# hyperpape/needle

Hardware: AMD Instinct MI355X
Metric: GB/s haystack scanned (10M x 256-char batch, DFA table walk) (higher is better)
Workload: dtype u8; 1 GPU; c2: '[0-9]+' containedIn() over 10000000 x 256 ASCII rows; rows_total=10000000, rows_per_gpu=10000000, row_chars=256, char_bytes=1, parallelism=row-shard x1, launch=eager

## Files before the change

### needle_amd/csrc/needle_device.h

```cpp
#pragma once
#include <stdint.h>

namespace needle {

enum Op : int { OP_MATCHES = 0, OP_CONTAINED_IN = 1, OP_FIND = 2 };

enum Mode : int {
    MODE_PACK = 0,
    MODE_TABLE8 = 1,
    MODE_TABLE16 = 2,
    MODE_GLOBAL = 3,
    MODE_HYBRID = 5,
    MODE_SPARSE = 6,
    MODE_PAIR = 4,
};

struct ProgHeader {
    uint32_t mode;
    uint32_t n_states;
    uint32_t n_cols;
    uint32_t start;
    uint32_t accept_lo;
    uint32_t root_accepting;
    uint32_t lds_bytes;
    uint32_t off_f;
    uint32_t pad_f;
    uint32_t pre_f;
    uint32_t off_cmap;
    uint32_t off_ptab;
    uint32_t off_pages;
    uint32_t off_table;
    uint32_t n_pages;
    uint32_t pad_col;
    uint32_t off_bcmap, off_bptab, off_bpages;
    uint32_t off_btable;
    uint8_t pack_off[8];
    uint32_t start_off, accept_off, ident_fn;
    uint32_t bpack_start_off, bpack_accept_off;
    uint32_t hot_bytes;
    uint32_t off_gtable;
    uint32_t off_bsp_bm;
    uint32_t off_bsp_base, off_bsp_edges;
    uint32_t sp_rec_base, sp_accept_rec, sp_rows_base;
    uint32_t sp_chains;
    uint32_t sp_pad_ident;
    uint32_t sp_dense, sp_records;
    uint32_t win_on, win_lo_e, win_hi_e;
    uint32_t fa_len_off, fa_dead_lo, fa_dead_n;
    uint32_t fa_dead_hi, sp_end_col4, sp_dead_row0, sp_len_cols;
    uint32_t fa_skip_lo;
    uint32_t flat_pages;
    uint32_t ft_on, ft_codes_off, ft_odd, ft_direct;
    uint32_t off_bpack;
};

struct ScanArgs {
    const uint8_t *rows;
    uint64_t n_rows;
    uint64_t stride_bytes;
    uint64_t total_bytes;
    uint32_t row_len;
    const uint32_t *lengths;
    const int32_t *from;
    const uint8_t *prog;
    ProgHeader hdr;
    const uint8_t *bprog;
    ProgHeader bhdr;
    int32_t fixed_len;
    uint32_t tiles_in_f_rows;
    uint64_t *bitmap;
    int32_t *start;
    int32_t *end;
    uint32_t *packed;
    uint32_t packed8;
    uint32_t *end_state;
    uint32_t short_window;
    uint32_t defer_max_live;
};

struct PackedArgs {
    ScanArgs s;
    const uint64_t *offsets;
    int32_t *overflow;
};

struct SpecArgs {
    const uint8_t *rows;
    uint64_t n_rows;
    uint64_t stride_bytes;
    uint32_t stripe_bytes;
    uint32_t spr;
    uint32_t char_width;
    uint32_t op;
    uint32_t row_len;
    const uint32_t *lengths;
    const uint8_t *gprog;
    ProgHeader hdr;
    uint32_t *slen;
    const uint32_t *spec_end_state;
    const int32_t *spec_last;
    const uint64_t *spec_bitmap;
    uint32_t *entry;
    uint32_t *entry_done;
    uint32_t *true_end_state;
    int32_t *true_last;
    int32_t *changed;
    uint64_t *bitmap;
    int32_t *end;
};

constexpr uint32_t kStripeBytes = 4096;
struct StripeArgs {
    const uint8_t *rows;
    uint64_t n_rows;
    uint64_t stride_bytes;
    uint32_t row_len;
    const uint32_t *lengths;
    const uint8_t *prog;
    ProgHeader hdr;
    uint32_t spr;
    uint32_t *fn;
    uint64_t *bitmap;
    uint32_t *cand;
    int32_t *cand_stripe;
    int32_t *end;
    int32_t *start;
    const uint8_t *bprog;
    ProgHeader bhdr;
    int32_t fixed_len;
    uint32_t op;
};

__host__ __device__ inline uint16_t pack8(int32_t s, int32_t e) {
    if (e < 0) return 0xFFFFu;
    const uint32_t len = (uint32_t)(e - s);
    return len > 255u ? (uint16_t)0xFFFEu : (uint16_t)(((uint32_t)s & 0xFFu) | len << 8);
}
constexpr uint32_t kPack16Over = 0xFFFEFFFFu;
constexpr uint16_t kPack8Over = 0xFFFDu;
__host__ __device__ inline uint32_t pack16_or_over(int32_t s, int32_t e) {
    if (e < 0) return 0xFFFFFFFFu;
    return e <= 65534 ? (((uint32_t)s & 0xFFFFu) | (uint32_t)e << 16) : kPack16Over;
}
__host__ __device__ inline uint16_t pack8_or_over(int32_t s, int32_t e) {
    if (e < 0) return 0xFFFFu;
    return e <= 256 ? pack8(s, e) : kPack8Over;
}
constexpr uint32_t kLdsF1 = 0, kLdsCmap1 = 0, kLdsTable1 = 512;
constexpr uint32_t kLdsCmapB1 = 512, kLdsPairTable1 = 1024;
constexpr uint32_t kLdsPtab2 = 0;
constexpr uint32_t kLdsPagesF2 = 2048, kLdsPages2Table = 512;
constexpr uint32_t kMaxPackPagesBytes = 96u * 1024u;

constexpr int kWavesPerBlock = 16;
constexpr uint32_t kMaxProgLdsBytes = 160u * 1024u - 4u * 64u * 64u;

}
```

### needle_amd/csrc/needle_kernels.hip

```cpp
#include "needle_walk.h"

namespace needle {

struct LaunchShape {
    int grid, waves, chb;
    size_t lds;
};
hipError_t launch_scan_matches(const ScanArgs &a, int cw, bool guard, LaunchShape sh, hipStream_t s);
hipError_t launch_scan_contained_in(const ScanArgs &a, int cw, bool guard, LaunchShape sh, hipStream_t s);
hipError_t launch_scan_find(const ScanArgs &a, int cw, bool guard, LaunchShape sh, hipStream_t s);

bool shape_for_program(const ProgHeader &h, int char_width, int *waves, int *chb, int *tiles_in_f_rows) {
    const size_t p = (h.lds_bytes + 15u) & ~15u;
    const size_t cap = 160u * 1024u;
    *tiles_in_f_rows = 0;
    static const char *force = getenv("NEEDLE_SHAPE");
    if (force) {
        int w = 0, c = 0;
        if (sscanf(force, "%dx%d", &w, &c) == 2 && (c == 64 || c == 128) && w >= 1 && w <= 16 && p + (size_t)w * 64 * c <= cap) {
            *waves = w;
            *chb = c;
            return true;
        }
    }
    if (h.mode == MODE_PACK && char_width == 1) {
        static const int min_waves = getenv("NEEDLE_PACK_WAVES") ? atoi(getenv("NEEDLE_PACK_WAVES")) : 14;
        for (int w = 16; w >= min_waves && w >= 5; --w)
            if (p + (size_t)(w - 4) * 8192u <= cap) {
                *waves = w;
                *chb = 128;
                *tiles_in_f_rows = 1;
                return true;
            }
    }
    static const int cand[8][2] = {{16, 128}, {12, 128}, {16, 64}, {14, 64}, {12, 64}, {10, 64}, {8, 64}, {4, 64}};
    for (const auto &c : cand) {
        if (p + (size_t)c[0] * 64 * c[1] <= cap) {
            *waves = c[0];
            *chb = c[1];
            return true;
        }
    }
    return false;
}

hipError_t launch_short_rows(int op, int char_width, const ScanArgs &a, int n_cus, hipStream_t stream);

hipError_t launch_scan(int op, int char_width, const ScanArgs &a_in, int n_cus, hipStream_t stream) {
    if (a_in.n_rows == 0) return hipSuccess;
    {
        static const int short_rows = getenv("NEEDLE_SHORT_ROWS") ? atoi(getenv("NEEDLE_SHORT_ROWS")) : 1;
        if (short_rows && a_in.stride_bytes <= 64 && a_in.hdr.mode != MODE_HYBRID && a_in.hdr.mode != MODE_SPARSE)
            return launch_short_rows(op, char_width, a_in, n_cus, stream);
    }
    ScanArgs a = a_in;
    LaunchShape sh;
    int in_f = 0;
    if (!shape_for_program(a.hdr, char_width, &sh.waves, &sh.chb, &in_f)) return hipErrorInvalidValue;
    a.tiles_in_f_rows = (uint32_t)in_f;
    const uint64_t n_groups = (a.n_rows + 63) >> 6;
    uint64_t blocks = (n_groups + sh.waves - 1) / sh.waves;
    static const int reserve = getenv("NEEDLE_RESERVE_CUS") ? atoi(getenv("NEEDLE_RESERVE_CUS")) : 0;
    if (reserve > 0 && n_cus > reserve + 8) n_cus -= reserve;
    if (blocks > (uint64_t)n_cus) blocks = (uint64_t)n_cus;
    sh.grid = (int)blocks;
    sh.lds = ((a.hdr.lds_bytes + 15u) & ~15u) + (size_t)(sh.waves - (in_f ? 4 : 0)) * 64 * sh.chb;
    static const int defer_env = getenv("NEEDLE_DEFER") ? atoi(getenv("NEEDLE_DEFER")) : 16;
    a.defer_max_live = 0;
    if (defer_env > 0 && defer_env <= 32 && !a.from && !a.end_state && a.n_rows < (1ull << 32)) a.defer_max_live = (uint32_t)defer_env;
    const bool guard = a.lengths != nullptr || a.from != nullptr || a.row_len == 0 ||
                       ((uint64_t)a.row_len * char_width) % sh.chb != 0;
    switch (op) {
    case OP_MATCHES: return launch_scan_matches(a, char_width, guard, sh, stream);
    case OP_CONTAINED_IN: return launch_scan_contained_in(a, char_width, guard, sh, stream);
    default: return launch_scan_find(a, char_width, guard, sh, stream);
    }
}

}
```

### needle_amd/csrc/needle_scan.h

```cpp
#pragma once
#include "needle_walk.h"

namespace needle {

template <int OP, int CW, int MODE, bool GUARD, int CHB, bool LEN = false>
__global__ __launch_bounds__(kWavesPerBlock * 64) void scan_kernel(const ScanArgs a) {
    using G = Geom<CHB>;
    constexpr bool POOL = MODE != MODE_PACK && CHB == 64;
    const int tid = threadIdx.x;
    const int lane = tid & 63;
    const int wave = __builtin_amdgcn_readfirstlane(tid >> 6);
    const int n_waves = blockDim.x >> 6;

    if ((uint32_t)(uintptr_t)(__attribute__((address_space(3))) unsigned char *)smem != 0u) __builtin_trap();
    for (uint32_t i = tid * 16u; i < a.hdr.lds_bytes; i += blockDim.x * 16u)
        *(u32x4 *)(smem + i) = *(const u32x4 *)(a.prog + i);
    __syncthreads();

    Walk wk;
    constexpr uint32_t ELEM = (MODE == MODE_TABLE16 || MODE == MODE_HYBRID) ? 2u : 1u;
    wk.ncols_e = a.hdr.n_cols * ELEM;
    wk.pad_e = (MODE == MODE_PACK) ? a.hdr.pad_f : a.hdr.pad_col * ELEM;
    wk.pre_e = (MODE == MODE_PACK) ? a.hdr.pre_f : (a.hdr.pad_col + 1u) * ELEM;
    wk.pad_b = wk.pre_b = 0;
    if (MODE == MODE_PAIR) {
        wk.ncols_e = a.hdr.n_cols * a.hdr.n_cols * 2u;
        wk.pad_e = a.hdr.pad_col * a.hdr.n_cols * 2u;
        wk.pre_e = (a.hdr.pad_col + 1u) * a.hdr.n_cols * 2u;
        wk.pad_b = a.hdr.pad_col * 2u;
        wk.pre_b = (a.hdr.pad_col + 1u) * 2u;
    }
    if (MODE == MODE_SPARSE) wk.pad_e = wk.pre_e = a.hdr.win_lo_e;
    wk.win_on = a.hdr.win_on;
    wk.win_lo = a.hdr.win_lo_e;
    wk.win_hi = a.hdr.win_hi_e;
    wk.dead_hi = OP == OP_FIND ? a.hdr.fa_dead_hi : 0u;
    wk.sp_chains = a.hdr.sp_chains;
    wk.sp_pad_ident = a.hdr.sp_pad_ident;
    wk.flat = (CW == 2 && (MODE == MODE_TABLE8 || MODE == MODE_TABLE16)) ? a.hdr.flat_pages : 0u;
    wk.table_off = a.hdr.off_table - (MODE == MODE_SPARSE ? 0u : a.hdr.win_lo_e);
    wk.lane4 = (uint32_t)(lane & 31) * 4u;
    wk.gtable = (const uint16_t *)(a.prog + (MODE == MODE_HYBRID ? a.hdr.off_gtable : a.hdr.off_table));
    if (MODE == MODE_HYBRID) wk.gtable = (const uint16_t *)((const uint8_t *)wk.gtable - a.hdr.win_lo_e);
    wk.hot_last = a.hdr.hot_bytes - 2u + a.hdr.win_lo_e;
    const uint32_t accept_lo = MODE == MODE_PACK ? a.hdr.accept_off : a.hdr.accept_lo;
    const uint32_t start_state = MODE == MODE_PACK ? a.hdr.start_off : a.hdr.start;

    Tile tile;
    {
        uint32_t base, row_stride;
        if (a.tiles_in_f_rows && wave < 4) {
            base = kLdsF1 + (uint32_t)wave * 64u * 256u + 128u;
            row_stride = 256u;
        } else {
            const uint32_t first = a.tiles_in_f_rows ? 4u : 0u;
            base = ((a.hdr.lds_bytes + 15u) & ~15u) + ((uint32_t)wave - first) * G::kTileBytes;
            row_stride = CHB;
        }
        tile.store_addr = base + (uint32_t)(lane / G::kPieces) * row_stride + (uint32_t)(lane % G::kPieces) * 16u;
        tile.store_step = G::kRowsPerInstr * row_stride;
        tile.row_addr = base + (uint32_t)lane * row_stride;
    }

    const uint64_t n_groups = (a.n_rows + 63) >> 6;
    const uint64_t wave_cnt = (uint64_t)gridDim.x * n_waves;
    uint64_t g = (uint64_t)blockIdx.x * n_waves + wave;
    if (g >= n_groups) return;

    const uint32_t q = (uint32_t)lane >> 4;
    const uint32_t p_in_row = (uint32_t)(lane % G::kPieces);
    const uint32_t row_in_instr = (uint32_t)(lane / G::kPieces);
    const uint32_t o_even = row_in_instr * (uint32_t)a.stride_bytes + 16u * (p_in_row ^ q);
    const uint32_t o_odd = CHB == 128 ? (row_in_instr * (uint32_t)a.stride_bytes + 16u * (p_in_row ^ q ^ 4u)) : o_even;
    const uint64_t load_step = (uint64_t)G::kRowsPerInstr * a.stride_bytes;

    constexpr int NT = (CHB == 64) ? 2 : 1;
    u32x4 R[NT][G::kInstrs];
    auto stage_and_fetch = [&](auto tc, bool do_fetch, uint64_t grp, uint32_t unit) __attribute__((always_inline)) {
        constexpr int T = decltype(tc)::value;
        if (!do_fetch) {
#pragma unroll
            for (int j = 0; j < G::kInstrs; ++j) store_piece(tile, j, R[T][j]);
            return;
        }
        const uint8_t *base = a.rows + (grp << 6) * a.stride_bytes + unit * (NT * CHB);
#pragma unroll
        for (int j = 0; j < G::kInstrs; ++j) {
            store_piece(tile, j, R[T][j]);
            asm volatile("" ::: "memory");
#pragma unroll
            for (int t = 0; t < NT; ++t) R[t][j] = load_row16<NT == 1>(base + t * CHB + j * load_step + ((j & 1) ? o_odd : o_even));
            asm volatile("" ::: "memory");
        }
    };
    auto fetch = [&](uint64_t grp, uint32_t unit) __attribute__((always_inline)) {
        const uint8_t *base = a.rows + (grp << 6) * a.stride_bytes + unit * (NT * CHB);
#pragma unroll
        for (int j = 0; j < G::kInstrs; ++j)
#pragma unroll
            for (int t = 0; t < NT; ++t) R[t][j] = load_row16<NT == 1>(base + t * CHB + j * load_step + ((j & 1) ? o_odd : o_even));
    };
    auto fetch_clamped = [&](uint64_t grp, uint32_t chunk) __attribute__((always_inline)) {
        const uint32_t last_r = (uint32_t)(a.n_rows - 1 - (grp << 6));
        const uint32_t stride = (uint32_t)a.stride_bytes;
        const uint8_t *gbase = a.rows + (grp << 6) * a.stride_bytes;
#pragma unroll
        for (int j = 0; j < G::kInstrs; ++j) {
            uint32_t r = (uint32_t)(j * G::kRowsPerInstr) + row_in_instr;
            const uint32_t kk = p_in_row ^ (uint32_t)G::swz((int)r);
            r = r < last_r ? r : last_r;
            uint32_t pb = chunk * CHB + kk * 16u;
            if (pb + 16u > stride) pb = stride - 16u;
            R[0][j] = load_row16<false>(gbase + (r * stride + pb));
        }
    };

    uint64_t my_row;
    bool row_ok;
    uint32_t len, n_chunks, st;
    int32_t last;
    int32_t cursor = 0;
    bool dead = false;
    u32x4 snapA = {0, 0, 0, 0}, snapB = {0, 0, 0, 0}, carry = {0, 0, 0, 0};
    int32_t snap_pi = 0;
    bool snapB_ok = true, carry_ok = true;
    uint32_t p_row = 0, p_ck = 0, p_st = 0;
    int32_t p_last = -1;
    uint64_t pool_mask = 0;
    auto begin_group = [&](uint64_t grp) __attribute__((always_inline)) {
        my_row = (grp << 6) + lane;
        row_ok = my_row < a.n_rows;
        len = 0;
        if (row_ok) len = a.lengths ? a.lengths[my_row] : a.row_len;
        const uint32_t max_len = GUARD ? wave_max(len) : a.row_len;
        n_chunks = (max_len * CW + CHB - 1) / CHB;
        if (n_chunks == 0) n_chunks = 1;
        st = start_state;
        if (GUARD && OP == OP_FIND && a.from) {
            cursor = row_ok ? a.from[my_row] : -1;
            dead = cursor < 0;
            if (dead) cursor = 0, st = 0;
        }
        snapB_ok = carry_ok = true;
        last = -1;
        if (OP == OP_FIND && a.hdr.root_accepting) last = ((uint32_t)cursor < len) ? cursor : 0;
    };

    auto walk_tile = [&](uint32_t idx0, uint32_t piece0) __attribute__((always_inline)) -> uint64_t {
        const uint32_t rem = len > idx0 ? len - idx0 : 0;
        const uint32_t skip = (uint32_t)cursor > idx0 ? (uint32_t)cursor - idx0 : 0;
        int32_t last_rel = -1;
        constexpr bool BIG = NEEDLE_BIG_ROLLED && (MODE == MODE_SPARSE || MODE == MODE_HYBRID);
        constexpr int kUnroll = BIG ? 1 : GUARD ? (OP == OP_FIND ? 1 : 2) : G::kPieces;
        constexpr int kUnrollSplit = BIG ? 1 : G::kPieces;
        constexpr int CPP = 16 / CW;
        u32x4 v = tile_piece<CHB>(tile, lane, 0);
        if (GUARD && NEEDLE_SPLIT_BOUNDARY) {
            const uint32_t n_in = rem / CPP;
            const uint32_t first_in = (skip + CPP - 1) / CPP;
            const bool cursor_cut = (skip % CPP != 0) && (skip / CPP < (uint32_t)G::kPieces);
            if (cursor_cut) {
                const uint32_t cp = skip / CPP;
                const u32x4 c = tile_piece<CHB>(tile, lane, (int)cp);
                const uint32_t w[4] = {c[0], c[1], c[2], c[3]};
                walk_piece<OP, CW, MODE, true>(wk, w, cp * CPP, rem, skip, accept_lo, st, last_rel);
            }
#pragma unroll kUnrollSplit
            for (int kk = 0; kk < G::kPieces; ++kk) {
                const uint32_t w[4] = {v[0], v[1], v[2], v[3]};
                if (kk + 1 < G::kPieces) v = tile_piece<CHB>(tile, lane, kk + 1);
                if ((uint32_t)kk >= first_in && (uint32_t)kk < n_in)
                    walk_piece<OP, CW, MODE, false>(wk, w, kk * CPP, 0, 0, accept_lo, st, last_rel);
            }
            if (n_in < (uint32_t)G::kPieces && rem % CPP != 0 && !(cursor_cut && skip / CPP == n_in)) {
                const u32x4 b = tile_piece<CHB>(tile, lane, (int)n_in);
                const uint32_t w[4] = {b[0], b[1], b[2], b[3]};
                walk_piece<OP, CW, MODE, true>(wk, w, n_in * CPP, rem, skip, accept_lo, st, last_rel);
            }
        } else {
        constexpr bool HIST = OP == OP_FIND && MODE == MODE_PACK && !GUARD;
        uint32_t acc_hist = 0;
#pragma unroll kUnroll
        for (int kk = 0; kk < G::kPieces; ++kk) {
            const uint32_t w[4] = {v[0], v[1], v[2], v[3]};
            if (kk + 1 < G::kPieces) v = tile_piece<CHB>(tile, lane, kk + 1);
            const uint32_t p0 = kk * CPP;
            walk_piece<OP, CW, MODE, GUARD, HIST>(wk, w, p0, rem, skip, accept_lo, st, last_rel, &acc_hist);
            if (HIST && ((kk + 1) * CPP) % 32 == 0) {
                const int32_t top = 31 - (int32_t)__builtin_clz(acc_hist | 1u);
                last_rel = acc_hist ? (int32_t)((kk + 1) * CPP - 32) + top + 1 : last_rel;
                acc_hist = 0;
            }
        }
        }
        if (OP == OP_FIND) {
            if (a.fixed_len < 0 && !LEN && !a.hdr.fa_len_off) {
                if (last_rel >= 0) {
                    const uint32_t pi = ((uint32_t)(last_rel - 1) * CW) >> 4;
                    snapA = tile_piece<CHB>(tile, lane, (int)pi);
                    const u32x4 before = tile_piece<CHB>(tile, lane, (int)(pi ? pi - 1 : 0));
                    snapB = pi ? before : carry;
                    snapB_ok = pi != 0u || carry_ok;
                    snap_pi = (int32_t)(piece0 + pi);
                }
                carry = tile_piece<CHB>(tile, lane, G::kPieces - 1);
            }
            last = last_rel >= 0 ? (int32_t)idx0 + last_rel : last;
        }
        bool live;
        if (OP == OP_CONTAINED_IN) live = st < accept_lo;
        else live = st > wk.dead_hi;
        if (GUARD) live = live && (idx0 + CHB / CW < len);
        return __ballot(live);
    };

    auto finish_rows = [&](uint64_t grp, auto pooled_c) __attribute__((always_inline)) {
        constexpr bool POOLED = decltype(pooled_c)::value;
        const KernargPtr ka = kernarg_here();
        uint64_t *const o_bitmap = kernarg_ptr<uint64_t>(ka, (uint32_t)offsetof(ScanArgs, bitmap));
        uint32_t *const o_end_state = kernarg_ptr<uint32_t>(ka, (uint32_t)offsetof(ScanArgs, end_state));
        bool res;
        if (OP == OP_FIND) res = row_ok && !dead && (last >= 0);
        else res = row_ok && (st >= accept_lo);
        if (!POOLED) {
            const uint64_t word = __ballot(res);
            if (lane == 0) {
                if (POOL) __hip_atomic_store(&o_bitmap[grp], word, __ATOMIC_RELAXED, __HIP_MEMORY_SCOPE_AGENT);
                else o_bitmap[grp] = word;
            }
        } else if (res) {
            __hip_atomic_fetch_or(&o_bitmap[my_row >> 6], 1ull << (my_row & 63), __ATOMIC_RELAXED, __HIP_MEMORY_SCOPE_AGENT);
        }
        if (o_end_state && row_ok) o_end_state[my_row] = st;
        if (OP != OP_FIND) return;
        int32_t s = -1;
        const int32_t e = res ? last : -1;
        if (a.fixed_len >= 0) {
            s = res ? last - a.fixed_len : -1;
        } else if (LEN || a.hdr.fa_len_off) {
            uint32_t pidx = st;
            if (MODE == MODE_SPARSE) {
                const uint32_t st_end = sparse_end<CW>(wk, st, st > wk.dead_hi, a.hdr.sp_end_col4);
                pidx = (st_end & 0xFFFFu) - a.hdr.sp_dead_row0;
            }
            s = res ? last - (int32_t)lds_u8(a.hdr.fa_len_off + pidx) : -1;
        } else {
            const uint8_t *rowp = a.rows + (row_ok ? my_row : 0) * a.stride_bytes;
            if (res) {
                *(lds_u32x4 *)(uintptr_t)(tile.row_addr) = snapB;
                *(lds_u32x4 *)(uintptr_t)(tile.row_addr + 16u) = snapA;
            }
            const uint32_t win_lo = snapB_ok ? 0u : 16u;
            const uint32_t win0 = (uint32_t)(snap_pi - 1) * 16u + win_lo;
            const int32_t lastb = backward_walk<CW>(a, res, last, cursor, tile.row_addr + win_lo, win0, 32u - win_lo, 0u, rowp);
            s = res ? lastb : -1;
        }
        if (row_ok) {
            uint32_t *const o_packed = kernarg_ptr<uint32_t>(ka, (uint32_t)offsetof(ScanArgs, packed));
            if (o_packed && kernarg_u32(ka, (uint32_t)offsetof(ScanArgs, packed8))) {
                ((uint16_t *)o_packed)[my_row] = pack8(s, e);
            } else if (o_packed) {
                o_packed[my_row] = ((uint32_t)s & 0xFFFFu) | ((uint32_t)e << 16);
            } else {
                kernarg_ptr<int32_t>(ka, (uint32_t)offsetof(ScanArgs, start))[my_row] = s;
                kernarg_ptr<int32_t>(ka, (uint32_t)offsetof(ScanArgs, end))[my_row] = e;
            }
        }
    };

    uint64_t last_group = n_groups - 1;
    {
        const uint64_t group_bytes = 64 * a.stride_bytes;
        const uint64_t safe = a.total_bytes >= (uint64_t)(NT * CHB) ? (a.total_bytes - NT * CHB) / group_bytes : 0;
        if (safe < last_group) last_group = safe;
    }
    auto defer_rows = [&](uint64_t live, uint32_t next_ck) __attribute__((always_inline)) {
        const bool is_live = (live >> lane) & 1ull;
        const uint32_t n_live = (uint32_t)__builtin_popcountll(live);
        const uint64_t free = ~pool_mask;
        const uint32_t q = __builtin_amdgcn_mbcnt_hi((uint32_t)(live >> 32), __builtin_amdgcn_mbcnt_lo((uint32_t)live, 0u));
        const uint32_t rf = __builtin_amdgcn_mbcnt_hi((uint32_t)(free >> 32), __builtin_amdgcn_mbcnt_lo((uint32_t)free, 0u));
        const uint32_t dest = is_live ? q : n_live + ((uint32_t)lane - q);
        const uint32_t nth_live = (uint32_t)__builtin_amdgcn_ds_permute((int)(dest << 2), lane);
        const bool take = ((free >> lane) & 1ull) && rf < n_live;
        const uint32_t src = (uint32_t)__builtin_amdgcn_ds_bpermute((int)((rf & 63u) << 2), (int)nth_live) << 2;
        const uint32_t t_row = (uint32_t)__builtin_amdgcn_ds_bpermute((int)src, (int)(uint32_t)my_row);
        const uint32_t t_st = (uint32_t)__builtin_amdgcn_ds_bpermute((int)src, (int)st);
        p_row = take ? t_row : p_row;
        p_st = take ? t_st : p_st;
        p_ck = take ? next_ck : p_ck;
        if (OP == OP_FIND) {
            const int32_t t_last = __builtin_amdgcn_ds_bpermute((int)src, last);
            p_last = take ? t_last : p_last;
        }
        pool_mask |= __ballot(take);
        row_ok = row_ok && !is_live;
    };

    auto pool_step = [&]() __attribute__((always_inline)) {
        const bool in_pool = (pool_mask >> lane) & 1ull;
        my_row = p_row;
        row_ok = in_pool;
        len = 0;
        if (in_pool) len = a.lengths ? a.lengths[p_row] : a.row_len;
        st = in_pool ? p_st : 0u;
        last = p_last;
        cursor = 0;
        dead = false;
        snap_pi = 1 << 24;
        snapB_ok = false;
        carry_ok = false;
        const uint32_t g_row = in_pool ? p_row : 0u;
        const uint32_t unit = in_pool ? p_ck / NT : 0u;
#pragma unroll
        for (int j = 0; j < G::kInstrs; ++j) {
            const uint32_t slot = (uint32_t)(j * G::kRowsPerInstr) + row_in_instr;
            const uint32_t srow = (uint32_t)__builtin_amdgcn_ds_bpermute((int)(slot << 2), (int)g_row);
            const uint32_t sunit = (uint32_t)__builtin_amdgcn_ds_bpermute((int)(slot << 2), (int)unit);
            const uint32_t kk = p_in_row ^ (uint32_t)G::swz((int)slot);
            const uint8_t *ptr = a.rows + (uint64_t)srow * a.stride_bytes + (uint64_t)sunit * (NT * CHB) + kk * 16u;
#pragma unroll
            for (int t = 0; t < NT; ++t) R[t][j] = load_row16<NT == 1>(ptr + t * CHB);
        }
        uint32_t n_ch = (len * CW + CHB - 1) / CHB;
        if (n_ch == 0) n_ch = 1;
        bool mine = in_pool;
        for (int t = 0; t < NT; ++t) {
#pragma unroll
            for (int j = 0; j < G::kInstrs; ++j) store_piece(tile, j, R[0][j]);
            const uint64_t live = walk_tile((p_ck + (uint32_t)t) * (CHB / CW), (p_ck + (uint32_t)t) * G::kPieces);
            carry_ok = true;
            const bool more = mine && ((live >> lane) & 1ull) && (p_ck + (uint32_t)t + 1u < n_ch);
            row_ok = mine && !more;
            pool_mask &= ~__ballot(row_ok);
            finish_rows(0, std::true_type{});
            mine = more;
            if (!mine) st = 0u;
            if (__ballot(mine) == 0ull) break;
            if (NT == 2) {
#pragma unroll
                for (int j = 0; j < G::kInstrs; ++j) R[0][j] = R[NT - 1][j];
            }
        }
        p_st = st;
        p_last = last;
        p_ck = in_pool ? p_ck + NT : 0u;
    };

    if (g < last_group) {
        uint32_t ck = 0;
        uint32_t pred_exit = 0xFFFFFFFFu;
        begin_group(g);
        fetch(g, 0);
        auto step = [&](auto tc) __attribute__((always_inline)) -> int {
            constexpr int T = decltype(tc)::value;
            const bool do_pf = (T == NT - 1) || (ck + 1 >= n_chunks) || (ck >= pred_exit);
            const bool pf_same = (T == NT - 1) && (ck + 1 < n_chunks) && (ck < pred_exit);
            const uint64_t pf_g = pf_same ? g : g + wave_cnt;
            stage_and_fetch(tc, do_pf && pf_g < last_group, pf_g, pf_same ? (ck + 1) / NT : 0u);
            asm volatile("" ::: "memory");
            const uint64_t live = walk_tile(ck * (CHB / CW), ck * G::kPieces);
            bool group_done = live == 0ull || (ck + 1 >= n_chunks);
            if (POOL && !group_done && T == NT - 1 && a.defer_max_live) {
                const uint32_t n_live = (uint32_t)__builtin_popcountll(live);
                if (n_live <= a.defer_max_live && n_live <= 64u - (uint32_t)__builtin_popcountll(pool_mask)) {
                    defer_rows(live, ck + 1);
                    group_done = true;
                }
            }
            if (!group_done) {
                if (do_pf && !pf_same) fetch(g, (ck + 1) / NT);
                ++ck;
                return 0;
            }
            finish_rows(g, std::false_type{});
            pred_exit = (ck + 1 < n_chunks) ? ck : 0xFFFFFFFFu;
            g += wave_cnt;
            return (!do_pf || pf_same) ? 3 : 1;
        };
        for (;;) {
            int r = step(std::integral_constant<int, 0>{});
            if (NT == 2 && r == 0) r = step(std::integral_constant<int, NT - 1>{});
            if (r == 0) continue;
            const bool more_groups = g < last_group;
            bool have_unit = r == 1;
            if (POOL) {
                const uint32_t keep = more_groups ? 64u - a.defer_max_live : 0u;
                while ((uint32_t)__builtin_popcountll(pool_mask) > keep) {
                    pool_step();
                    have_unit = false;
                }
            }
            if (!more_groups) break;
            if (!have_unit) fetch(g, 0);
            ck = 0;
            begin_group(g);
        }
    }
    for (; g < n_groups; g += wave_cnt) {
        begin_group(g);
        for (uint32_t ck = 0; ck < n_chunks; ++ck) {
            fetch_clamped(g, ck);
            stage_and_fetch(std::integral_constant<int, 0>{}, false, 0, 0);
            if (walk_tile(ck * (CHB / CW), ck * G::kPieces) == 0ull) break;
        }
        finish_rows(g, std::false_type{});
    }
}

struct LaunchShape {
    int grid, waves, chb;
    size_t lds;
};

template <int OP, int CW, int MODE, bool GUARD, int CHB, bool LEN>
static hipError_t launch_one(const ScanArgs &a, LaunchShape sh, hipStream_t stream) {
    auto k = scan_kernel<OP, CW, MODE, GUARD, CHB, LEN>;
    static thread_local uint64_t configured = 0;
    if (hipError_t e = allow_full_lds((const void *)k, configured); e != hipSuccess) return e;
    hipLaunchKernelGGL(k, dim3(sh.grid), dim3(sh.waves * 64), sh.lds, stream, a);
    return hipGetLastError();
}

template <int OP, int CW, int MODE, bool GUARD, bool LEN>
static hipError_t launch_h(const ScanArgs &a, LaunchShape sh, hipStream_t s) {
    return sh.chb == 128 ? launch_one<OP, CW, MODE, GUARD, 128, LEN>(a, sh, s) : launch_one<OP, CW, MODE, GUARD, 64, LEN>(a, sh, s);
}

template <int OP, int CW, int MODE, bool LEN = false>
static hipError_t launch_g(const ScanArgs &a, bool guard, LaunchShape sh, hipStream_t s) {
    if constexpr (OP == OP_FIND && !LEN && (MODE == MODE_TABLE8 || MODE == MODE_TABLE16 || MODE == MODE_SPARSE || MODE == MODE_PAIR)) {
        if (a.hdr.fa_len_off) return launch_g<OP, CW, MODE, true>(a, guard, sh, s);
    }
    return guard ? launch_h<OP, CW, MODE, true, LEN>(a, sh, s) : launch_h<OP, CW, MODE, false, LEN>(a, sh, s);
}

template <int OP, int CW>
static hipError_t launch_m(const ScanArgs &a, bool guard, LaunchShape sh, hipStream_t s) {
    switch (a.hdr.mode) {
    case MODE_PACK: return launch_g<OP, CW, MODE_PACK>(a, guard, sh, s);
    case MODE_TABLE8: return launch_g<OP, CW, MODE_TABLE8>(a, guard, sh, s);
    case MODE_TABLE16: return launch_g<OP, CW, MODE_TABLE16>(a, guard, sh, s);
    case MODE_PAIR: return CW == 1 ? launch_g<OP, 1, MODE_PAIR>(a, guard, sh, s) : hipErrorInvalidValue;
    case MODE_HYBRID: return launch_g<OP, CW, MODE_HYBRID>(a, guard, sh, s);
    case MODE_SPARSE: return launch_g<OP, CW, MODE_SPARSE>(a, guard, sh, s);
    default: return launch_g<OP, CW, MODE_GLOBAL>(a, guard, sh, s);
    }
}

template <int OP>
static hipError_t launch_c(const ScanArgs &a, int cw, bool guard, LaunchShape sh, hipStream_t s) {
    return cw == 1 ? launch_m<OP, 1>(a, guard, sh, s) : launch_m<OP, 2>(a, guard, sh, s);
}

}
```

### needle_amd/csrc/needle_tuning.cpp

```cpp
#include <stdio.h>
#include <stdlib.h>
#include <string.h>
#include <string>
#include "../../include/needle_hip.h"

namespace {
struct Switch {
    const char *name, *dflt, *scope, *effect;
};
const Switch kSwitches[] = {
    {"NEEDLE_PREFILTER", "1", "layout", "n-gram candidate filter in front of the automaton (needle_ngram.hip): 0 never, 1 for automata in the compressed form, 2 for every LDS-table automaton that allows one"},
    {"NEEDLE_PREFILTER_LEVEL2", "1", "layout", "0: no second-level window (a candidate's 5-byte window looked up in a second bitmap before the automaton runs on it)"},
    {"NEEDLE_PREFILTER_UTF16", "1", "layout", "0: UTF-16 rows never take a filter kernel (patterns on one page of the BMP: the byte program's, text narrowed as it is loaded; several pages: the wide filter)"},
    {"NEEDLE_PACKED_DIRECT_ABOVE", "2147483647", "debug", "packed rows behind the n-gram filter (needle_ngram_packed.h): a 64-row group whose span has more chars than this is walked row by row inside the filter kernel instead of being filtered (the default is the limit of the kernel's 32-bit stream positions; lower values let tests reach that path; answers are the same)"},
    {"NEEDLE_PREFILTER_PACKED", "1", "layout", "0: packed row batches (needle_*_packed_dev) never take the n-gram filter kernel (needle_ngram_packed.h): every packed call walks the plain packed kernel, as with needle_pattern_set_prefilter(OFF)"},
    {"NEEDLE_PREFILTER_WIDE", "1", "layout", "0: UTF-16 rows of patterns on several pages of the BMP never take the wide filter (windows of four 16-bit code units, needle_ngram.h ngram_piece16); NEEDLE_PREFILTER_UTF16=0 switches it off too"},
    {"NEEDLE_PREFILTER_UNBOUNDED", "1", "layout", "0: find() of patterns without bounded match lengths never runs behind the n-gram filter (whose verified candidates find their starts by backward walks)"},
    {"NEEDLE_PREFILTER_STRIDE", "4", "layout", "largest window stride the n-gram filter may choose (2: never 4 -- keeps the second-level window for patterns whose shortest match is 7 chars)"},
    {"NEEDLE_PREFILTER_WATCH", "1", "layout", "0: the filter kernel is never suspended (the flood watch: after a launch that saw more than 16 candidates per KiB of text the program's next 32 .. 1024 calls take the ordinary scan kernel)"},
    {"NEEDLE_FIND_LENGTHS", "1", "layout", "find() by the lengths automaton (start = end - length, no backward walk): 0 never (forward + backward walks), 1 where the ordinary program is an LDS table, 2 also instead of a pair table"},
    {"NEEDLE_FIND_LENGTHS_SPARSE", "1", "layout", "0: compressed-form automata keep the two walks"},
    {"NEEDLE_FIND_LENGTHS_PAIR", "1", "layout", "0: pair-table automata keep the two walks"},
    {"NEEDLE_FIND_ALL_LENGTHS", "1", "layout", "find-all's starts: 0 by backward walks, 1 by the lengths automaton where it fits the LDS as a plain table, 2 also in its compressed form (big dictionaries; measured: no faster)"},
    {"NEEDLE_FIND_ALL_LOCKSTEP", "1", "layout", "0: find-all never takes the lock-step kernel (the find-all transducer, needle_find_all_ls.hip); patterns that have one keep the per-lane one-pass kernel"},
    {"NEEDLE_FIND_ALL_RUNS", "1", "layout", "0: find-all of run patterns (`[0-9]+`: no bounded match length) never takes the lock-step kernel with the run transducer; they keep the per-lane one-pass kernel and its backward walks"},
    {"NEEDLE_FIND_ALL_FILTER", "1", "layout", "0: find-all never runs behind the n-gram candidate filter (dictionaries whose find() does keep the one-pass find-all kernel)"},
    {"NEEDLE_FIND_ALL_WINDOW", "1", "layout", "0: the find-all kernel's lengths program keeps column-map lookups instead of window addressing"},
    {"NEEDLE_FIND_ALL_DEFER", "1", "layout", "0: find-all (two-walk form) finds each start as the match is found instead of deferring them to the row's end"},
    {"NEEDLE_FIND_ALL_ROUNDS", "0", "layout", "1: find-all as rounds of needle_find_next_dev (one pass over the batch per match rank) instead of the one-pass kernel"},
    {"NEEDLE_FIND_ALL_SHAPE", "(by LDS footprint)", "layout", "\"<waves>x<tile bytes>\" workgroup shape of the find-all kernel"},
    {"NEEDLE_SPARSE", "1", "layout", "0: automata larger than the LDS skip the compressed form (dense rows + exception records) and fall to hot rows + HBM table"},
    {"NEEDLE_SPARSE_ROOM", "98304", "size", "LDS bytes the compressed form may take"},
    {"NEEDLE_HYBRID", "1", "layout", "0: no hot-rows form either: plain HBM table"},
    {"NEEDLE_WINDOW", "1", "layout", "0: column-map lookups instead of window addressing (clamped char = column offset)"},
    {"NEEDLE_FLAT_MAP", "1", "layout", "0: UTF-16 rows of LDS-table automata always use the compact two-level page map instead of the flat 64 KB one (one column lookup per char)"},
    {"NEEDLE_BTABLE_LDS_MAX", "8192", "size", "largest dense backward table of find() that rides in the forward program's LDS image when 16 waves of tiles still fit beside it (2048: round 4's rule)"},
    {"NEEDLE_PAIR_MAX_BYTES", "98304", "size", "largest pair table ([state][col][col] uint16, two chars per lookup); 0: never"},
    {"NEEDLE_MAX_PROG_LDS", "(device limit)", "size", "LDS bytes an automaton may take (tests lower it to force the HBM-table mode)"},
    {"NEEDLE_SHAPE", "(by LDS footprint)", "layout", "\"<waves>x<tile bytes>\" workgroup shape of the tiled scan kernel"},
    {"NEEDLE_PACK_WAVES", "14", "layout", "fewest waves a packed-mode workgroup may have before 128-byte tiles are given up"},
    {"NEEDLE_SHORT_ROWS", "1", "layout", "0: rows of at most 64 bytes take the tiled kernel instead of the register-resident one"},
    {"NEEDLE_SHORT_WGS", "2", "layout", "workgroups per CU of the short-row kernel"},
    {"NEEDLE_DEFER", "16", "layout", "survivor pool: a 64-row group with at most this many unresolved rows hands them to the wave's pool (0: off; at most 32)"},
    {"NEEDLE_RESERVE_CUS", "0", "layout", "CUs left free by the persistent scan launch (for an RCCL gather running beside it)"},
    {"NEEDLE_LONG_ROWS", "-1", "layout", "few long rows: -1 by shape, 0 never take the stripe paths, 1 always"},
    {"NEEDLE_STRIPE_CAND", "1", "layout", "0: stripe-path find() re-walks every stripe instead of only the last accepting one"},
    {"NEEDLE_MULTI_PACK16", "1", "layout", "needle_multi_scan find(): 0 peers send int32 start / end, 1 one dword per row, 2 also for shards on the root's device (tests)"},
    {"NEEDLE_MULTI_NO_RCCL", "0", "layout", "1: needle_multi gathers by peer copies instead of RCCL"},
    {"NEEDLE_HOST_CHUNK_BYTES", "2147483648", "size", "device bytes one chunk of a host batch may take"},
    {"NEEDLE_HOST_RESULT_BYTES", "536870912", "size", "device bytes the results of one find-all host chunk may take"},
    {"NEEDLE_SCRATCH_KEEP_MB", "512", "size", "freed scratch memory the library's pool keeps for the next call (needle_trim_scratch hands back the rest)"},
    {"NEEDLE_SPARSE_DEBUG", "(unset)", "debug", "prints the compressed form's sizing to stderr"},
    {"NEEDLE_ML_DEBUG", "(unset)", "debug", "prints why a pattern has no lengths automaton"},
    {"NEEDLE_COMPILE_TIMING", "(unset)", "debug", "prints where needle_compile's time goes (subset construction, pruning, minimisation per automaton)"},
    {"NEEDLE_DEBUG_NFA", "(unset)", "debug", "dumps the forward Thompson program of needle_compile"},
    {"NEEDLE_DICT", "0", "measurement build", "two 64-row sets per wave for big automata (needle_dict.hip): 1 compressed form, 2 also uint16 tables"},
    {"NEEDLE_NG_DBG", "0", "measurement build", "n-gram filter kernel time breakdown (drops candidates / skips walks: timing only)"},
    {"NEEDLE_NG_STAMPS", "0", "measurement build", "1: every n-gram filter launch is synchronised and prints where its waves' shader cycles went (text wait / probes / queue / second level / verify walks / group ends)"},
    {"NEEDLE_DEBUG_NO_BACKWARD", "(unset)", "measurement build", "find() with start := end (the bound the lengths automaton was built to reach)"},
};
}

extern "C" int needle_tuning_info(char *buf, size_t cap, size_t *needed) {
    std::string out = "name\tdefault\tcurrent\tscope\teffect\n";
    for (const Switch &s : kSwitches) {
        const char *cur = getenv(s.name);
        out += s.name;
        out += '\t';
        out += s.dflt;
        out += '\t';
        out += cur ? cur : "";
        out += '\t';
        out += s.scope;
        out += '\t';
        out += s.effect;
        out += '\n';
    }
    if (needed) *needed = out.size() + 1;
    if (buf && cap) {
        const size_t n = out.size() < cap - 1 ? out.size() : cap - 1;
        memcpy(buf, out.data(), n);
        buf[n] = 0;
    }
    return NEEDLE_OK;
}
```

Measured before the change: 6388 GB/s.

## Interleave two row groups per wave in packed scan with per-row fetch skipping

In packed mode for matches/containedIn with 128-byte tiles, each wave now alternates between two 64-row groups. It stages one group's tile and issues the next fetch for the other group before walking, so memory latency overlaps the DFA walk. Buffer loads for rows that already have a verdict get an out-of-range offset bit, so those lines are never fetched and HBM traffic on finished rows drops. The cost is more register pressure and extra control flow, and an env switch can turn the skipping off.

New measurement: 7089 GB/s, median of 6. 11.0% higher.

```diff
diff --git a/needle_amd/csrc/needle_device.h b/needle_amd/csrc/needle_device.h
--- a/needle_amd/csrc/needle_device.h
+++ b/needle_amd/csrc/needle_device.h
@@ -76,6 +76,7 @@
     uint32_t *end_state;
     uint32_t short_window;
     uint32_t defer_max_live;
+    uint32_t pack_skip;
 };
 
 struct PackedArgs {
diff --git a/needle_amd/csrc/needle_kernels.hip b/needle_amd/csrc/needle_kernels.hip
--- a/needle_amd/csrc/needle_kernels.hip
+++ b/needle_amd/csrc/needle_kernels.hip
@@ -68,6 +68,8 @@
     static const int defer_env = getenv("NEEDLE_DEFER") ? atoi(getenv("NEEDLE_DEFER")) : 16;
     a.defer_max_live = 0;
     if (defer_env > 0 && defer_env <= 32 && !a.from && !a.end_state && a.n_rows < (1ull << 32)) a.defer_max_live = (uint32_t)defer_env;
+    static const int pack_skip = getenv("NEEDLE_PACK_SKIP") ? atoi(getenv("NEEDLE_PACK_SKIP")) : 1;
+    a.pack_skip = pack_skip != 0;
     const bool guard = a.lengths != nullptr || a.from != nullptr || a.row_len == 0 ||
                        ((uint64_t)a.row_len * char_width) % sh.chb != 0;
     switch (op) {
diff --git a/needle_amd/csrc/needle_scan.h b/needle_amd/csrc/needle_scan.h
--- a/needle_amd/csrc/needle_scan.h
+++ b/needle_amd/csrc/needle_scan.h
@@ -7,6 +7,7 @@
 __global__ __launch_bounds__(kWavesPerBlock * 64) void scan_kernel(const ScanArgs a) {
     using G = Geom<CHB>;
     constexpr bool POOL = MODE != MODE_PACK && CHB == 64;
+    constexpr bool TWO = MODE == MODE_PACK && OP != OP_FIND && CHB == 128;
     const int tid = threadIdx.x;
     const int lane = tid & 63;
     const int wave = __builtin_amdgcn_readfirstlane(tid >> 6);
@@ -99,6 +100,27 @@
         for (int j = 0; j < G::kInstrs; ++j)
 #pragma unroll
             for (int t = 0; t < NT; ++t) R[t][j] = load_row16<NT == 1>(base + t * CHB + j * load_step + ((j & 1) ? o_odd : o_even));
+    };
+    constexpr uint32_t kDropBit = 0x80000000u;
+    auto stage_and_fetch_rows = [&](bool do_fetch, uint64_t grp, uint32_t chunk, uint64_t rows) __attribute__((always_inline)) {
+        if (!do_fetch) {
+#pragma unroll
+            for (int j = 0; j < G::kInstrs; ++j) store_piece(tile, j, R[0][j]);
+            return;
+        }
+        const uint8_t *base = a.rows + (grp << 6) * a.stride_bytes + chunk * CHB;
+        const __amdgpu_buffer_rsrc_t rsrc = __builtin_amdgcn_make_buffer_rsrc((void *)base, 0, (int)kDropBit, 0x00020000);
+        const uint64_t drop = ~rows >> row_in_instr;
+        const uint32_t drop_lo = (uint32_t)drop, drop_hi = (uint32_t)(drop >> 32);
+#pragma unroll
+        for (int j = 0; j < G::kInstrs; ++j) {
+            store_piece(tile, j, R[0][j]);
+            asm volatile("" ::: "memory");
+            const uint32_t d = ((j < 4 ? drop_lo : drop_hi) << (31 - 8 * (j & 3))) & kDropBit;
+            R[0][j] = __builtin_amdgcn_raw_buffer_load_b128(rsrc, (int)(d | ((j & 1) ? o_odd : o_even)), (int)(j * (uint32_t)load_step),
+                                                            NEEDLE_NT_LOADS ? 2  : 0);
+            asm volatile("" ::: "memory");
+        }
     };
     auto fetch_clamped = [&](uint64_t grp, uint32_t chunk) __attribute__((always_inline)) {
         const uint32_t last_r = (uint32_t)(a.n_rows - 1 - (grp << 6));
@@ -135,6 +157,7 @@
         const uint32_t max_len = GUARD ? wave_max(len) : a.row_len;
         n_chunks = (max_len * CW + CHB - 1) / CHB;
         if (n_chunks == 0) n_chunks = 1;
+        if (TWO && GUARD) n_chunks = (uint32_t)__builtin_amdgcn_readfirstlane((int)n_chunks);
         st = start_state;
         if (GUARD && OP == OP_FIND && a.from) {
             cursor = row_ok ? a.from[my_row] : -1;
@@ -347,7 +370,50 @@
         p_ck = in_pool ? p_ck + NT : 0u;
     };
 
-    if (g < last_group) {
+    if constexpr (TWO) {
+        if (a.stride_bytes > (1u << 24)) last_group = 0;
+        if (g < last_group) {
+            const uint64_t keep = a.pack_skip ? 0ull : ~0ull;
+            uint64_t g_o = g + wave_cnt, next_g = g + 2 * wave_cnt, live_o = ~0ull;
+            uint32_t ck = 0, ck_o = 0, st_o = start_state, len_o = 0, nch_o = 1;
+            if (g_o < last_group) {
+                begin_group(g_o);
+                st_o = st, len_o = len, nch_o = n_chunks;
+            }
+            begin_group(g);
+            fetch(g, 0);
+            for (;;) {
+                const bool two = g_o < last_group;
+                const bool pf_same = !two && ck + 1 < n_chunks;
+                stage_and_fetch_rows(two || pf_same, two ? g_o : g, two ? ck_o : ck + 1, two ? (live_o | keep) : ~0ull);
+                asm volatile("" ::: "memory");
+                const uint64_t live = walk_tile(ck * (CHB / CW), ck * G::kPieces);
+                const bool group_done = live == 0ull || ck + 1 >= n_chunks;
+                if (group_done) {
+                    my_row = (g << 6) + lane;
+                    row_ok = true;
+                    finish_rows(g, std::false_type{});
+                    g = next_g;
+                    next_g += wave_cnt;
+                    ck = 0;
+                    if (g < last_group) begin_group(g);
+                } else {
+                    ++ck;
+                }
+                if (two) {
+                    const uint64_t tg = g; g = g_o; g_o = tg;
+                    const uint32_t tc = ck; ck = ck_o; ck_o = tc;
+                    const uint32_t ts = st; st = st_o; st_o = ts;
+                    const uint32_t tl = len; len = len_o; len_o = tl;
+                    const uint32_t tn = n_chunks; n_chunks = nch_o; nch_o = tn;
+                    live_o = group_done ? ~0ull : live;
+                } else if (g >= last_group) {
+                    break;
+                }
+            }
+            g = g < g_o ? g : g_o;
+        }
+    } else if (g < last_group) {
         uint32_t ck = 0;
         uint32_t pred_exit = 0xFFFFFFFFu;
         begin_group(g);
diff --git a/needle_amd/csrc/needle_tuning.cpp b/needle_amd/csrc/needle_tuning.cpp
--- a/needle_amd/csrc/needle_tuning.cpp
+++ b/needle_amd/csrc/needle_tuning.cpp
@@ -39,6 +39,7 @@
     {"NEEDLE_MAX_PROG_LDS", "(device limit)", "size", "LDS bytes an automaton may take (tests lower it to force the HBM-table mode)"},
     {"NEEDLE_SHAPE", "(by LDS footprint)", "layout", "\"<waves>x<tile bytes>\" workgroup shape of the tiled scan kernel"},
     {"NEEDLE_PACK_WAVES", "14", "layout", "fewest waves a packed-mode workgroup may have before 128-byte tiles are given up"},
+    {"NEEDLE_PACK_SKIP", "1", "layout", "0: packed-mode matches() / containedIn() fetch every 128-byte line of every row of an unfinished 64-row group instead of only the lines of rows still without a verdict (same kernel and fetch order; for A/B runs)"},
     {"NEEDLE_SHORT_ROWS", "1", "layout", "0: rows of at most 64 bytes take the tiled kernel instead of the register-resident one"},
     {"NEEDLE_SHORT_WGS", "2", "layout", "workgroups per CU of the short-row kernel"},
     {"NEEDLE_DEFER", "16", "layout", "survivor pool: a 64-row group with at most this many unresolved rows hands them to the wave's pool (0: off; at most 32)"},
```
